# PaulMayer123/IMS-Toucan-Prosody-Variance

Hardware: AMD Instinct MI355X
Metric: mel-frames/sec + vocoder RTF @24kHz, batch=32, 1/2/4/8 MI355X (higher is better)
Workload: dtype bf16

## Files before the change

ims-toucan-prosody-variance_amd/csrc/common.h:

```cpp
#pragma once
#include <hip/hip_runtime.h>
#include <stdint.h>
#include <stdio.h>

#include "../../include/toucan_tts.h"

namespace tts {

void set_error(const char* fmt, ...);

#define TTS_CHECK_ARG(cond, ...)   \
  do {                             \
    if (!(cond)) {                 \
      tts::set_error(__VA_ARGS__); \
      return TTS_E_ARG;            \
    }                              \
  } while (0)

inline int launch_status(const char* what) {
  hipError_t e = hipGetLastError();
  if (e != hipSuccess) {
    set_error("%s: %s", what, hipGetErrorString(e));
    return TTS_E_LAUNCH;
  }
  return TTS_OK;
}

inline hipError_t raise_lds_limit(const void* kernel, unsigned long long& mask) {
  int dev = 0;
  (void)hipGetDevice(&dev);
  const unsigned long long bit = 1ull << (dev & 63);
  if (mask & bit) return hipSuccess;
  int room = 160 * 1024;
  hipFuncAttributes attr;
  if (hipFuncGetAttributes(&attr, kernel) == hipSuccess) room -= (int)attr.sharedSizeBytes;
  else (void)hipGetLastError();
  const hipError_t e = hipFuncSetAttribute(kernel, hipFuncAttributeMaxDynamicSharedMemorySize, room);
  if (e == hipSuccess) mask |= bit;
  else (void)hipGetLastError();
  return e;
}

struct WavenetCond {
  const float* g;
  int ld_g;
  const void* wc;
  int wc_n;
  int col0;
  const float* bc;
};
int wavenet_layer_cond(const TtsWavenetDesc& d, const WavenetCond& c, hipStream_t st);

typedef float f32x16 __attribute__((ext_vector_type(16)));
typedef float f32x4 __attribute__((ext_vector_type(4)));
typedef short bf16x8 __attribute__((ext_vector_type(8)));

__device__ __forceinline__ unsigned short f32_to_bf16(float f) {
  const __bf16 b = (__bf16)f;
  return __builtin_bit_cast(unsigned short, b);
}
__device__ __forceinline__ float bf16_to_f32(unsigned short u) { return __builtin_bit_cast(float, (unsigned int)u << 16); }

typedef _Float16 f16x2 __attribute__((ext_vector_type(2)));
typedef __bf16 bf16x2 __attribute__((ext_vector_type(2)));
typedef _Float16 f16x8 __attribute__((ext_vector_type(8)));
typedef float f32x2 __attribute__((ext_vector_type(2)));
__device__ __forceinline__ unsigned short f32_to_f16(float f) { return __builtin_bit_cast(unsigned short, (_Float16)f); }
__device__ __forceinline__ float f16_to_f32(unsigned short u) { return (float)__builtin_bit_cast(_Float16, u); }
template <bool F16>
__device__ __forceinline__ unsigned short to16(float f) {
  if constexpr (F16) return f32_to_f16(f);
  else return f32_to_bf16(f);
}
template <bool F16>
__device__ __forceinline__ float from16(unsigned short u) {
  if constexpr (F16) return f16_to_f32(u);
  else return bf16_to_f32(u);
}
template <bool F16>
__device__ __forceinline__ unsigned int pack16(float lo, float hi) {
  const f32x2 v = {lo, hi};
  if constexpr (F16) return __builtin_bit_cast(unsigned int, __builtin_convertvector(v, f16x2));
  else return __builtin_bit_cast(unsigned int, __builtin_convertvector(v, bf16x2));
}
__device__ __forceinline__ float load16(unsigned short u, bool f16) { return f16 ? f16_to_f32(u) : bf16_to_f32(u); }
__device__ __forceinline__ unsigned short store16(float v, bool f16) { return f16 ? f32_to_f16(v) : f32_to_bf16(v); }

template <bool F16>
__device__ __forceinline__ f32x16 mfma16(bf16x8 a, bf16x8 b, f32x16 c) {
  if constexpr (F16) return __builtin_amdgcn_mfma_f32_32x32x16_f16(__builtin_bit_cast(f16x8, a), __builtin_bit_cast(f16x8, b), c, 0, 0, 0);
  else return __builtin_amdgcn_mfma_f32_32x32x16_bf16(a, b, c, 0, 0, 0);
}

#define TTS_GLOAD128(dst_, ptr_) asm volatile("global_load_dwordx4 %0, %1, off" : "=v"(dst_) : "v"(ptr_) : "memory")
#define TTS_GLOAD32(dst_, ptr_) asm volatile("global_load_dword %0, %1, off" : "=v"(dst_) : "v"(ptr_) : "memory")
#define TTS_WAIT_VM(n_) asm volatile("s_waitcnt vmcnt(%0)" ::"n"(n_) : "memory")
#define TTS_PIN(r_) asm volatile("" : "+v"(r_))

__device__ __forceinline__ float sigmoidf_(float v) { return 1.0f / (1.0f + __expf(-v)); }

__device__ __forceinline__ float wave_sum(float v) {
#pragma unroll
  for (int o = 32; o > 0; o >>= 1) v += __shfl_xor(v, o, 64);
  return v;
}

__device__ __forceinline__ float wave_max(float v) {
#pragma unroll
  for (int o = 32; o > 0; o >>= 1) v = fmaxf(v, __shfl_xor(v, o, 64));
  return v;
}

}
```

ims-toucan-prosody-variance_amd/csrc/pipeline.hip:

```cpp
#include <algorithm>
#include <cmath>
#include <cstdlib>
#include <cstring>
#include <string>
#include <unordered_map>
#include <utility>
#include <vector>

#include "common.h"
#include "../../include/toucan_prosody.h"
#include "../../include/toucan_prosody_curves.h"
#include "../../include/toucan_score.h"

namespace tts {

const char* conv1d_wide_reject(const TtsConvDesc& d);

namespace {

constexpr int ATT = 192, HEADS = 4, DK = 48;

struct Dev {
  void* p = nullptr;
  int64_t shape[4] = {0, 0, 0, 0};
// ... 1095 lines not shown

int pipeline_teacher_forced(Handle* h, const float* gold_pitch, const float* gold_energy, const int* gold_dur, float* pred_log_dur,
                            float* pred_pitch, float* pred_energy, int* frames_out, hipStream_t st) {
  TTS_CHECK_ARG(h && h->enc, "tts_teacher_forced: run tts_encoder first");
  TTS_CHECK_RESOLVED(h, "tts_teacher_forced");
  TTS_CHECK_ARG(gold_pitch && gold_energy && gold_dur && pred_log_dur && pred_pitch && pred_energy, "tts_teacher_forced: null pointer");
  h->split_mode = 2;
  h->tab_which = 0;
  const Acoustic& m = h->acoustic;
  const int R = h->lp.total;
  if (h->cfg.multispeaker) TTS_TRY(cln_prepare(h, st));
  TTS_TRY(predictor(h, m.pitch, pred_pitch, st));
  TTS_TRY(predictor(h, m.energy, pred_energy, st));
  TTS_TRY(predictor(h, m.duration, pred_log_dur, st));
  TTS_TRY(hip_ok(hipMemcpyAsync(h->pitch, gold_pitch, (size_t)R * 4, hipMemcpyDeviceToDevice, st), "gold pitch"));
  TTS_TRY(hip_ok(hipMemcpyAsync(h->energy, gold_energy, (size_t)R * 4, hipMemcpyDeviceToDevice, st), "gold energy"));
  TTS_TRY(hip_ok(hipMemcpyAsync(h->dur, gold_dur, (size_t)R * 4, hipMemcpyDeviceToDevice, st), "gold durations"));
  return regulate(h, gold_dur, true, frames_out, st);
}

int pipeline_decoder(Handle* h, hipStream_t st) {
  TTS_CHECK_ARG(h && h->dec, "tts_decoder: run tts_control_and_regulate first");
  TTS_CHECK_RESOLVED(h, "tts_decoder");
  h->split_mode = 1;
  h->tab_which = 0;
  TTS_TRY(conformer(h, 1, h->dec, h->lf, h->frame, st));
  TTS_ALLOC(mel0, h->frame, float, (size_t)h->lf.total * 80);
  h->mel0 = mel0;
  h->mel = nullptr;
  return conv(h, h->acoustic.feat_out, T2(h->dec, ATT), T2(mel0, 80), h->lf, st);
}

int pipeline_postnet(Handle* h, hipStream_t st) {
  TTS_CHECK_ARG(h && h->mel0, "tts_postnet: run tts_decoder first");
  TTS_CHECK_RESOLVED(h, "tts_postnet");
  h->split_mode = 1;
  h->tab_which = 0;
  const Layout& l = h->lf;
  const int RF = l.total;
  Arena& a = h->frame;
  TTS_ALLOC(x, a, float, (size_t)RF * 256);
  TTS_ALLOC(y, a, float, (size_t)RF * 256);
  TTS_ALLOC(y80, a, float, (size_t)RF * 80);
  const long long wsn = std::max<long long>(1, tts_groupnorm_workspace_floats(l.n(), l.max_len, 32));
  TTS_ALLOC(gws, a, float, wsn);
  const int *sb, *se;
  TTS_TRY(bounds_of(h, l, st, &sb, &se));
  const float* src = h->mel0;
  int ld = 80;
  for (int i = 0; i < 5; ++i) {
    const auto& p = h->acoustic.postnet[i];
    if (i < 4) {
      TTS_TRY(conv(h, p.conv, T2(const_cast<float*>(src), ld), T2(x, 256), l, st));
      TTS_TRY(tts_groupnorm(x, 256, y, 256, p.g, p.b, 256, 32, 1e-5f, 1, nullptr, 0, sb, se, l.n(), l.max_len, gws, st));
      src = y;
      ld = 256;
    } else {
      TTS_TRY(conv(h, p.conv, T2(const_cast<float*>(src), ld), T2(y80, 80), l, st));
      TTS_TRY(tts_groupnorm(y80, 80, h->cat, 80 + ATT, p.g, p.b, 80, 20, 1e-5f, 0, h->mel0, 80, sb, se, l.n(), l.max_len, gws, st));
    }
  }
  h->mel = h->cat;
  h->have_flow = false;
  return TTS_OK;
}

int pipeline_postflow(Handle* h, const float* z_noise, hipStream_t st) {
  TTS_CHECK_ARG(h && h->mel == h->cat && h->cat, "tts_postflow: run tts_postnet first");
  TTS_CHECK_ARG(z_noise, "tts_postflow: z_noise is required");
  TTS_CHECK_RESOLVED(h, "tts_postflow");
  h->split_mode = 1;
  h->tab_which = 0;
  const Layout ls = h->lf.halved();
  const int RF = h->lf.total, RS = RF / 2;
  Arena& a = h->frame;
  const int b16 = bits16(h);
  const Acoustic& m = h->acoustic;
  TTS_ALLOC(g, a, float, (size_t)RF * ATT);
  TTS_TRY(conv(h, m.g_proj, T2(h->cat, 80 + ATT), T2(g, ATT), h->lf, st));
  TTS_ALLOC(x, a, float, (size_t)RS * 160);
  TTS_TRY(hip_ok(hipMemcpyAsync(x, z_noise, (size_t)RS * 160 * 4, hipMemcpyDeviceToDevice, st), "flow noise"));
  TTS_ALLOC(hs, a, float, (size_t)RS * 2 * ATT);
  const bool fused = !postflow_cond_buffer(h);
  float* hs2 = nullptr;
  TileTab t64;
  if (fused) {
    hs2 = arena_alloc<float>(a, (size_t)RS * 2 * ATT);
    if (!hs2) {
      set_error("tts_postflow: workspace exhausted");
      return TTS_E_ARG;
    }
    TTS_TRY(tiles_of(h, ls, 64, st, &t64));
  }
  char* acts = nullptr;
  float* cond = nullptr;
  if (!fused) {
    acts = arena_alloc<char>(a, (size_t)RS * ATT * (b16 / 8));
    cond = arena_alloc<float>(a, (size_t)RS * 8 * ATT);
    if (!acts || !cond) {
      set_error("tts_postflow: workspace exhausted");
      return TTS_E_ARG;
    }
  }
  float* skip = hs + ATT;
  double live_rows = 0;
  for (int n : ls.lengths) live_rows += n;
  for (int b = 17; b >= 0; --b) {
    const auto& f = m.flow[b];
    const ConvW& cnd = f.cond;
    TTS_TRY(conv(h, f.start, T2(x, 160), T2(hs, 2 * ATT), ls, st));
    if (!fused) TTS_TRY(conv(h, cnd, T2(g, 2 * ATT), T2(cond, 8 * ATT), ls, st));
    float* cur = hs;
    for (int i = 0; i < 4; ++i) {
      const ConvW &inl = m.flowgrp[b / 4].inl[i], &rs = m.flowgrp[b / 4].res_skip[i];
      if (fused) {
        float* nxt = cur == hs ? hs2 : hs;
        TtsWavenetDesc w;
        memset(&w, 0, sizeof(w));
        w.hs_in = cur; w.ld_in = 2 * ATT; w.hs_out = nxt; w.ld_out = 2 * ATT;
        w.w1 = inl.w16; w.b1 = inl.bias; w.w2 = rs.w16; w.b2 = rs.bias;
        w.cout2 = rs.cout; w.compute = inl.compute16;
        w.tiles = t64.dev; w.n_tiles = t64.n; w.tile_rows = 64;
        TTS_CHECK_ARG(cnd.w16 && cnd.mode == TTS_MODE_LINEAR && cnd.compute16 == inl.compute16 && cnd.cin == 2 * ATT && cnd.cin_pad == 2 * ATT && cnd.cout == 8 * ATT &&
                          cnd.taps == 1 && cnd.wn >= 8 * ATT,
                      "tts_postflow: flow.%d.cond is not a 16-bit 1-tap 384 -> 1536 conv", b);
        const WavenetCond wc = {g, 2 * ATT, cnd.w16, cnd.wn, i * 2 * ATT, cnd.bias};
        TTS_TRY(prof_launch(h, "wavenet_layer", 2.0 * live_rows * (ATT * 5 * 2 * ATT + 2 * ATT * 2 * ATT + (double)ATT * rs.cout),
                            live_rows * 4.0 * (2 * ATT + rs.cout + 2 * ATT) + 2.0 * (5 * ATT * 2 * ATT + 2 * ATT * 2 * ATT + ATT * rs.cout),
                            live_rows * rs.cout, st, [&] { return wavenet_layer_cond(w, wc, st); }));
        cur = nxt;
        continue;
      }
      ConvOpt oi;
      oi.preadd = cond + (size_t)i * 2 * ATT;
      oi.ld_preadd = 8 * ATT;
      TTS_TRY(conv(h, inl, T2(hs, 2 * ATT), T2(acts, ATT, b16), ls, st, oi));
      ConvOpt orr;
      orr.accumulate = true;
      TTS_TRY(conv(h, rs, T2(acts, ATT, b16), i < 3 ? T2(hs, 2 * ATT) : T2(skip, 2 * ATT), ls, st, orr));
    }
    ConvOpt oe;
    oe.aux = x + 80;
    oe.ld_aux = 160;
    oe.fp32_only = true;
    TTS_TRY(conv(h, f.end, T2(cur + ATT, 2 * ATT), T2(x + 80, 160), ls, st, oe));
    TTS_TRY(tts_glow_invconv_actnorm(x, 160, RS, 160, f.winv, f.an_bias, f.an_logs, st));
  }
  h->mel = x;
  h->have_flow = true;
  return TTS_OK;
}

struct ArenaRewind {
  Arena& a;
  size_t off;
  explicit ArenaRewind(Arena& a_) : a(a_), off(a_.off) {}
  ~ArenaRewind() { a.off = off; }
};

int pipeline_postflow_nll(Handle* h, const float* gold, int ld_gold, float* loss, float* row_parts, float* z_out, hipStream_t st) {
  TTS_CHECK_ARG(h, "tts_postflow_nll: null handle");
  TTS_CHECK_ARG(!is16(h), "tts_postflow_nll: fp32 handles only (this one was created with precision %d)", h->cfg.precision);
  TTS_CHECK_ARG(find(h, "flow.logdet") && find(h, "flow.0.wfwd") && find(h, "flow.0.end_ml.w"),
                "tts_postflow_nll: the forward weights flow.<b>.wfwd, flow.<b>.end_ml and flow.logdet were not loaded (tts_load_weights; "
                "NativePipeline(..., scoring=True) uploads them)");
  TTS_CHECK_ARG(h->mel == h->cat && h->cat, "tts_postflow_nll: run tts_postnet first");
  TTS_CHECK_ARG(gold && ld_gold >= 80 && loss, "tts_postflow_nll: null gold_mel / loss_out, or row stride %d < 80", ld_gold);
  TTS_CHECK_RESOLVED(h, "tts_postflow_nll");
  const Acoustic& m = h->acoustic;
  TTS_CHECK_ARG(m.scoring, "tts_postflow_nll: the forward weights were not resolved: run tts_encoder again");
  h->split_mode = 1;
  h->tab_which = 0;
  const Layout ls = h->lf.halved();
  const int RF = h->lf.total, RS = RF / 2, B = h->lf.n();
  long long live_rows = 0;
  for (int n : ls.lengths) live_rows += n;
  const size_t ml_bytes = ((size_t)RS * 160 * 4 + 255) & ~(size_t)255, ld_bytes = ((size_t)RS * 8 + 255) & ~(size_t)255;
  TTS_TRY(arena_reserve(h->nll, ml_bytes + ld_bytes, st));
  TTS_ALLOC(ml, h->nll, float, (size_t)RS * 160);
  TTS_ALLOC(row_logdet, h->nll, double, RS);
  TTS_TRY(hip_ok(hipMemsetAsync(h->nll.base, 0, ml_bytes + ld_bytes, st), "tts_postflow_nll: clear scratch"));
  void* tab;
  TTS_TRY(table_of(h, layout_key(h->lf, -2), st, [&] {
    std::vector<int> host(3 * (size_t)B);
    for (int u = 0; u < B; ++u) {
      host[u] = ls.begins[u];
      host[B + u] = ls.lengths[u];
      host[2 * B + u] = h->lf.lengths[u];
    }
    return host;
  }, &tab, nullptr));
  const int* utt = static_cast<const int*>(tab);
  Arena& a = h->frame;
  ArenaRewind rewind(a);
  TTS_ALLOC(x, a, float, (size_t)RS * 160);
  TTS_TRY(hip_ok(hipMemcpy2DAsync(x, 80 * 4, gold, (size_t)ld_gold * 4, 80 * 4, RF, hipMemcpyDeviceToDevice, st), "tts_postflow_nll: gold mel"));
  if (live_rows > 0) {
    TTS_ALLOC(g, a, float, (size_t)RF * ATT);
    TTS_TRY(conv(h, m.g_proj, T2(h->cat, 80 + ATT), T2(g, ATT), h->lf, st));
    TTS_ALLOC(hs, a, float, (size_t)RS * 2 * ATT);
    TTS_ALLOC(acts, a, float, (size_t)RS * ATT);
    TTS_ALLOC(cond, a, float, (size_t)RS * 8 * ATT);
    float* skip = hs + ATT;
    TTS_TRY(tts_glow_forward_rows(x, 160, RS, nullptr, 0, nullptr, m.flow_fwd[0].wfwd, m.flow[0].an_bias, m.flow[0].an_logs, st));
    for (int b = 0; b < 18; ++b) {
      const auto& f = m.flow[b];
      TTS_TRY(conv(h, f.start, T2(x, 160), T2(hs, 2 * ATT), ls, st));
      TTS_TRY(conv(h, f.cond, T2(g, 2 * ATT), T2(cond, 8 * ATT), ls, st));
      for (int i = 0; i < 4; ++i) {
        const ConvW &inl = m.flowgrp[b / 4].inl[i], &rs = m.flowgrp[b / 4].res_skip[i];
        ConvOpt oi;
        oi.preadd = cond + (size_t)i * 2 * ATT;
        oi.ld_preadd = 8 * ATT;
        TTS_TRY(conv(h, inl, T2(hs, 2 * ATT), T2(acts, ATT), ls, st, oi));
        ConvOpt orr;
        orr.accumulate = true;
        TTS_TRY(conv(h, rs, T2(acts, ATT), i < 3 ? T2(hs, 2 * ATT) : T2(skip, 2 * ATT), ls, st, orr));
      }
      ConvOpt oe;
      oe.fp32_only = true;
      TTS_TRY(conv(h, m.flow_fwd[b].end_ml, T2(skip, 2 * ATT), T2(ml, 160), ls, st, oe));
      const bool last = b == 17;
      TTS_TRY(tts_glow_forward_rows(x, 160, RS, ml, 160, row_logdet, last ? nullptr : m.flow_fwd[b + 1].wfwd, last ? nullptr : m.flow[b + 1].an_bias,
                                    last ? nullptr : m.flow[b + 1].an_logs, st));
    }
  }
  TTS_TRY(tts_glow_nll_reduce(x, 160, row_logdet, utt, utt + B, utt + 2 * B, B, m.flow_logdet, loss, row_parts, st));
  if (z_out) TTS_TRY(hip_ok(hipMemcpyAsync(z_out, x, (size_t)RS * 160 * 4, hipMemcpyDeviceToDevice, st), "tts_postflow_nll: z_out"));
// ... 369 lines not shown
```

ims-toucan-prosody-variance_amd/csrc/wavenet.hip:

```cpp
#include "common.h"

namespace tts {

namespace {
constexpr int WN_H = 192;
constexpr int WN_BM = 64;
constexpr int WN_TAPS = 5;
constexpr int WN_XP = WN_H + 8;
constexpr int WN_G = 2 * WN_H;
constexpr int WN_GP = WN_G + 8;
constexpr int WN_STEPS1 = WN_TAPS * (WN_H / 16);
constexpr int WN_STEPSC = WN_G / 16;
constexpr int WN_STEPS2 = WN_H / 16;
constexpr int WN_DEPTH = 4;
constexpr int WN_L = 4;
constexpr size_t WN_XS_BYTES = ((size_t)(WN_BM + WN_TAPS - 1) * WN_XP * 2 + 255) / 256 * 256;
constexpr size_t WN_GS_BYTES = (size_t)WN_BM * WN_GP * 2;
static_assert(WN_STEPS1 % WN_DEPTH == 0 && WN_STEPSC % WN_DEPTH == 0 && WN_STEPS2 % WN_DEPTH == 0 && (WN_H / 16) % WN_DEPTH == 0,
              "a block of WN_DEPTH k-steps stays inside one tap and one product");
}

template <bool F16, bool FUSED>
__global__ __launch_bounds__(256) void wavenet_layer_kernel(const TtsWavenetDesc d, const WavenetCond cd) {
  extern __shared__ __attribute__((aligned(16))) unsigned char lds_raw[];
// ... 166 lines not shown
          }
        } else {
          const float4 ea = *reinterpret_cast<const float4*>(cr + c), eg = *reinterpret_cast<const float4*>(cr + WN_H + c);
          pa[0] = ea.x; pa[1] = ea.y; pa[2] = ea.z; pa[3] = ea.w;
          pg[0] = eg.x; pg[1] = eg.y; pg[2] = eg.z; pg[3] = eg.w;
        }
        const float bav[4] = {ba.x, ba.y, ba.z, ba.w}, bgv[4] = {bg.x, bg.y, bg.z, bg.w};
        float v[4];
#pragma unroll
        for (int q = 0; q < 4; ++q) {
          const float av = aa[4 * rq + q] + bav[q] + pa[q], gvv = ag[4 * rq + q] + bgv[q] + pg[q];
          const float th = 2.0f * __builtin_amdgcn_rcpf(1.0f + __expf(-2.0f * av)) - 1.0f;
          v[q] = th * __builtin_amdgcn_rcpf(1.0f + __expf(-gvv));
        }
        *reinterpret_cast<uint2*>(xs + t * WN_XP + c) = make_uint2(pack16<F16>(v[0], v[1]), pack16<F16>(v[2], v[3]));
      }
    };
    constexpr int CZ = FUSED ? 1 : 0;
    gate(acc[0], acc[2], accc[0 * CZ], accc[2 * CZ], P0, fP);
    gate(acc[1], acc[3], accc[1 * CZ], accc[3 * CZ], P0, fQ);
    gate(acc[4], acc[5], accc[4 * CZ], accc[5 * CZ], P1, fP);
#pragma unroll
    for (int j = 0; j < 6; ++j)
#pragma unroll
      for (int r = 0; r < 16; ++r) acc[j][r] = 0.0f;
  }
  publish();
  xload(xP, xQ, xs, WN_XP);
#pragma unroll 1
  for (int base = 0; base < WN_STEPS2; base += WN_DEPTH) {
    if (base == WN_STEPS2 - WN_DEPTH) {
      q0 -= qs; q1 -= qs; q2 -= qs; q3 -= qs;
      qs = 0;
    }
#pragma unroll
    for (int u = 0; u < WN_DEPTH; ++u) {
      const bf16x8 cP = xP, cQ = xQ;
      const int s1 = base + u + 1 < WN_STEPS2 ? base + u + 1 : WN_STEPS2 - 1;
      xload(xP, xQ, xs + s1 * 16, WN_XP);
      arrive(u);
      u32x4 wf[3];
#pragma unroll
      for (int i = 0; i < 3; ++i) wf[i] = wr[u][i];
      acc[0] = mfma16<F16>(__builtin_bit_cast(bf16x8, wf[0]), cP, acc[0]);
      acc[1] = mfma16<F16>(__builtin_bit_cast(bf16x8, wf[0]), cQ, acc[1]);
      acc[2] = mfma16<F16>(__builtin_bit_cast(bf16x8, wf[1]), cP, acc[2]);
      if (n2 == 384) {
        acc[3] = mfma16<F16>(__builtin_bit_cast(bf16x8, wf[1]), cQ, acc[3]);
        acc[4] = mfma16<F16>(__builtin_bit_cast(bf16x8, wf[2]), cP, acc[4]);
        acc[5] = mfma16<F16>(__builtin_bit_cast(bf16x8, wf[2]), cQ, acc[5]);
      }
      request(u);
    }
  }
  TTS_WAIT_VM(0);
#pragma unroll
  for (int u = 0; u < WN_DEPTH; ++u) {
    TTS_PIN(wr[u][0]);
    TTS_PIN(wr[u][1]);
    TTS_PIN(wr[u][2]);
    TTS_PIN(wr[u][3]);
  }
  {
    const int col0 = n2 == 384 ? 0 : WN_H;
    auto store_block = [&](const f32x16& a, int cb, int f) __attribute__((always_inline)) {
      const int row = tile.row0 + f * 32 + lrow;
      if (row >= tile.seq_end) return;
      const float* ir = d.hs_in + (size_t)row * d.ld_in + col0;
      float* orow = d.hs_out + (size_t)row * d.ld_out + col0;
#pragma unroll
      for (int rq = 0; rq < 4; ++rq) {
        const int c = cb * 32 + 8 * rq + 4 * lk;
        const float4 b = *reinterpret_cast<const float4*>(d.b2 + c), x = *reinterpret_cast<const float4*>(ir + c);
        *reinterpret_cast<float4*>(orow + c) = make_float4((a[4 * rq] + b.x) + x.x, (a[4 * rq + 1] + b.y) + x.y, (a[4 * rq + 2] + b.z) + x.z, (a[4 * rq + 3] + b.w) + x.w);
      }
    };
    store_block(acc[0], cb0, fP);
    store_block(acc[1], cb0, fQ);
    store_block(acc[2], cb1, fP);
    if (n2 == 384) {
      store_block(acc[3], cb1, fQ);
      store_block(acc[4], cb2, fP);
      store_block(acc[5], cb2, fQ);
    }
  }
}

namespace {
int wavenet_launch(const TtsWavenetDesc& d, const WavenetCond* c, hipStream_t st) {
  TTS_CHECK_ARG(d.hs_in && d.hs_out && d.w1 && d.b1 && d.w2 && d.b2 && d.tiles, "wavenet_layer: null pointer");
  TTS_CHECK_ARG(d.hs_in != d.hs_out, "wavenet_layer: the hidden state cannot be updated in place (the 5-tap conv reads neighbouring tiles)");
  TTS_CHECK_ARG(d.cout2 == 384 || d.cout2 == 192, "wavenet_layer: res/skip width %d (384, or 192 for the last layer)", d.cout2);
  TTS_CHECK_ARG(d.compute == TTS_COMPUTE_BF16 || d.compute == TTS_COMPUTE_F16, "wavenet_layer: 16-bit MFMA configurations only (compute %d)", d.compute);
  TTS_CHECK_ARG(d.tile_rows == WN_BM, "wavenet_layer: tile table must use %d rows, got %d", WN_BM, d.tile_rows);
  TTS_CHECK_ARG((d.ld_in & 3) == 0 && (d.ld_out & 3) == 0 && ((uintptr_t)d.hs_in & 15) == 0 && ((uintptr_t)d.hs_out & 15) == 0 && ((uintptr_t)d.w1 & 15) == 0 &&
                    ((uintptr_t)d.w2 & 15) == 0 && ((uintptr_t)d.b1 & 15) == 0 && ((uintptr_t)d.b2 & 15) == 0,
                "wavenet_layer: rows and weights must be 16-byte aligned");
  if (c) {
    TTS_CHECK_ARG(c->g && c->wc && c->bc, "wavenet_layer: null conditioning pointer");
    TTS_CHECK_ARG(c->ld_g >= WN_G && (c->ld_g & 3) == 0 && c->col0 >= 0 && (c->col0 & 31) == 0 && c->col0 + 2 * WN_H <= c->wc_n,
                  "wavenet_layer: conditioning columns %d .. of %d, row stride %d", c->col0, c->wc_n, c->ld_g);
    TTS_CHECK_ARG(((uintptr_t)c->g & 15) == 0 && ((uintptr_t)c->wc & 15) == 0 && ((uintptr_t)c->bc & 15) == 0, "wavenet_layer: conditioning operands must be 16-byte aligned");
  } else {
    TTS_CHECK_ARG(d.cond, "wavenet_layer: null pointer");
    TTS_CHECK_ARG((d.ld_cond & 3) == 0 && ((uintptr_t)d.cond & 15) == 0, "wavenet_layer: rows and weights must be 16-byte aligned");
  }
  if (d.n_tiles == 0) return TTS_OK;
  const bool f16 = d.compute == TTS_COMPUTE_F16;
  const WavenetCond none = {nullptr, 0, nullptr, 0, 0, nullptr};
  if (c) {
    const size_t lds = WN_XS_BYTES + WN_GS_BYTES;
    static unsigned long long raised[2] = {0, 0};
    const void* k = f16 ? reinterpret_cast<const void*>(wavenet_layer_kernel<true, true>) : reinterpret_cast<const void*>(wavenet_layer_kernel<false, true>);
    if (raise_lds_limit(k, raised[f16 ? 1 : 0]) != hipSuccess) {
      set_error("wavenet_layer: raising the dynamic LDS limit failed");
      return TTS_E_LAUNCH;
    }
    if (f16) hipLaunchKernelGGL((wavenet_layer_kernel<true, true>), dim3(d.n_tiles), dim3(256), lds, st, d, *c);
    else hipLaunchKernelGGL((wavenet_layer_kernel<false, true>), dim3(d.n_tiles), dim3(256), lds, st, d, *c);
  } else {
    if (f16) hipLaunchKernelGGL((wavenet_layer_kernel<true, false>), dim3(d.n_tiles), dim3(256), WN_XS_BYTES, st, d, none);
    else hipLaunchKernelGGL((wavenet_layer_kernel<false, false>), dim3(d.n_tiles), dim3(256), WN_XS_BYTES, st, d, none);
  }
  return launch_status("wavenet_layer");
}
}

int wavenet_layer(const TtsWavenetDesc& d, hipStream_t st) { return wavenet_launch(d, nullptr, st); }

int wavenet_layer_cond(const TtsWavenetDesc& d, const WavenetCond& c, hipStream_t st) { return wavenet_launch(d, &c, st); }

}

extern "C" int tts_wavenet_layer(const TtsWavenetDesc* d, tts_stream_t stream) {
  if (!d) {
    tts::set_error("tts_wavenet_layer: null descriptor");
    return TTS_E_ARG;
  }
  return tts::wavenet_layer(*d, reinterpret_cast<hipStream_t>(stream));
}
```

Before: 595,300.

## Fuse flow start conv and four WaveNet layers into one halo-tiled block kernel

Replaces the per-layer WaveNet launches (start conv plus four conditioned layers with ping-pong hidden buffers) with a single kernel per flow step. Each block computes 64 rows and stores the middle 48, relying on an 8-row halo on each side to cover the receptive field of the four 5-tap convs. The hidden state stays in registers and LDS across layers, and only the skip output is written to global memory. This removes the intermediate hidden-state round trips and launch overhead. In exchange it recomputes the halo rows (16 of every 64, about a third extra work per output row) and raises register and LDS pressure.

```diff
diff --git a/ims-toucan-prosody-variance_amd/csrc/common.h b/ims-toucan-prosody-variance_amd/csrc/common.h
--- a/ims-toucan-prosody-variance_amd/csrc/common.h
+++ b/ims-toucan-prosody-variance_amd/csrc/common.h
@@ -50,6 +50,20 @@
   const float* bc;
 };
 int wavenet_layer_cond(const TtsWavenetDesc& d, const WavenetCond& c, hipStream_t st);
+
+struct WavenetBlock {
+  const float* x; int ld_x;
+  float* skip; int ld_skip;
+  const void* w0; int w0_n; const float* b0;
+  const void* w1[4]; const float* b1[4];
+  const void* w2[4]; const float* b2[4];
+  const float* g; int ld_g;
+  const void* wc; int wc_n; const float* bc;
+  const TtsTile* tiles; int n_tiles; int tile_rows;
+  int compute;
+};
+int wavenet_block(const WavenetBlock& d, hipStream_t st);
+int wavenet_block_tile_rows();
 
 typedef float f32x16 __attribute__((ext_vector_type(16)));
 typedef float f32x4 __attribute__((ext_vector_type(4)));
diff --git a/ims-toucan-prosody-variance_amd/csrc/pipeline.hip b/ims-toucan-prosody-variance_amd/csrc/pipeline.hip
--- a/ims-toucan-prosody-variance_amd/csrc/pipeline.hip
+++ b/ims-toucan-prosody-variance_amd/csrc/pipeline.hip
@@ -1201,16 +1201,8 @@
   TTS_TRY(hip_ok(hipMemcpyAsync(x, z_noise, (size_t)RS * 160 * 4, hipMemcpyDeviceToDevice, st), "flow noise"));
   TTS_ALLOC(hs, a, float, (size_t)RS * 2 * ATT);
   const bool fused = !postflow_cond_buffer(h);
-  float* hs2 = nullptr;
-  TileTab t64;
-  if (fused) {
-    hs2 = arena_alloc<float>(a, (size_t)RS * 2 * ATT);
-    if (!hs2) {
-      set_error("tts_postflow: workspace exhausted");
-      return TTS_E_ARG;
-    }
-    TTS_TRY(tiles_of(h, ls, 64, st, &t64));
-  }
+  TileTab tblk;
+  if (fused) TTS_TRY(tiles_of(h, ls, wavenet_block_tile_rows(), st, &tblk));
   char* acts = nullptr;
   float* cond = nullptr;
   if (!fused) {
@@ -1227,29 +1219,33 @@
   for (int b = 17; b >= 0; --b) {
     const auto& f = m.flow[b];
     const ConvW& cnd = f.cond;
-    TTS_TRY(conv(h, f.start, T2(x, 160), T2(hs, 2 * ATT), ls, st));
-    if (!fused) TTS_TRY(conv(h, cnd, T2(g, 2 * ATT), T2(cond, 8 * ATT), ls, st));
-    float* cur = hs;
-    for (int i = 0; i < 4; ++i) {
+    if (!fused) {
+      TTS_TRY(conv(h, f.start, T2(x, 160), T2(hs, 2 * ATT), ls, st));
+      TTS_TRY(conv(h, cnd, T2(g, 2 * ATT), T2(cond, 8 * ATT), ls, st));
+    }
+    if (fused) {
+      TTS_CHECK_ARG(f.start.w16 && f.start.mode == TTS_MODE_LINEAR && f.start.compute16 == cnd.compute16 && f.start.cin == 80 && f.start.taps == 1 && f.start.wn >= ATT,
+                    "tts_postflow: flow.%d.start is not a 16-bit 1-tap 80 -> 192 conv", b);
+      TTS_CHECK_ARG(cnd.w16 && cnd.mode == TTS_MODE_LINEAR && cnd.cin == 2 * ATT && cnd.cin_pad == 2 * ATT && cnd.cout == 8 * ATT && cnd.taps == 1 && cnd.wn >= 8 * ATT,
+                    "tts_postflow: flow.%d.cond is not a 16-bit 1-tap 384 -> 1536 conv", b);
+      WavenetBlock w;
+      memset(&w, 0, sizeof(w));
+      w.x = x; w.ld_x = 160; w.skip = skip; w.ld_skip = 2 * ATT;
+      w.w0 = f.start.w16; w.w0_n = f.start.wn; w.b0 = f.start.bias;
+      w.g = g; w.ld_g = 2 * ATT; w.wc = cnd.w16; w.wc_n = cnd.wn; w.bc = cnd.bias;
+      w.tiles = tblk.dev; w.n_tiles = tblk.n; w.tile_rows = wavenet_block_tile_rows();
+      w.compute = cnd.compute16;
+      for (int i = 0; i < 4; ++i) {
+        const ConvW &inl = m.flowgrp[b / 4].inl[i], &rs = m.flowgrp[b / 4].res_skip[i];
+        TTS_CHECK_ARG(inl.w16 && rs.w16 && inl.compute16 == cnd.compute16 && rs.cout == (i < 3 ? 2 * ATT : ATT), "tts_postflow: flow.%d layer %d is not a 16-bit WaveNet layer", b, i);
+        w.w1[i] = inl.w16; w.b1[i] = inl.bias; w.w2[i] = rs.w16; w.b2[i] = rs.bias;
+      }
+      TTS_TRY(prof_launch(h, "wavenet_block", 2.0 * live_rows * (80.0 * ATT + 4.0 * (ATT * 5 * 2 * ATT + 2 * ATT * 2 * ATT) + 3.0 * ATT * 2 * ATT + (double)ATT * ATT),
+                          live_rows * 4.0 * (80 + ATT + 2 * ATT) + 2.0 * (80.0 * ATT + 4.0 * (5 * ATT * 2 * ATT + 2 * ATT * 2 * ATT) + 3.0 * ATT * 2 * ATT + (double)ATT * ATT),
+                          live_rows * ATT, st, [&] { return wavenet_block(w, st); }));
+    }
+    for (int i = 0; i < 4 && !fused; ++i) {
       const ConvW &inl = m.flowgrp[b / 4].inl[i], &rs = m.flowgrp[b / 4].res_skip[i];
-      if (fused) {
-        float* nxt = cur == hs ? hs2 : hs;
-        TtsWavenetDesc w;
-        memset(&w, 0, sizeof(w));
-        w.hs_in = cur; w.ld_in = 2 * ATT; w.hs_out = nxt; w.ld_out = 2 * ATT;
-        w.w1 = inl.w16; w.b1 = inl.bias; w.w2 = rs.w16; w.b2 = rs.bias;
-        w.cout2 = rs.cout; w.compute = inl.compute16;
-        w.tiles = t64.dev; w.n_tiles = t64.n; w.tile_rows = 64;
-        TTS_CHECK_ARG(cnd.w16 && cnd.mode == TTS_MODE_LINEAR && cnd.compute16 == inl.compute16 && cnd.cin == 2 * ATT && cnd.cin_pad == 2 * ATT && cnd.cout == 8 * ATT &&
-                          cnd.taps == 1 && cnd.wn >= 8 * ATT,
-                      "tts_postflow: flow.%d.cond is not a 16-bit 1-tap 384 -> 1536 conv", b);
-        const WavenetCond wc = {g, 2 * ATT, cnd.w16, cnd.wn, i * 2 * ATT, cnd.bias};
-        TTS_TRY(prof_launch(h, "wavenet_layer", 2.0 * live_rows * (ATT * 5 * 2 * ATT + 2 * ATT * 2 * ATT + (double)ATT * rs.cout),
-                            live_rows * 4.0 * (2 * ATT + rs.cout + 2 * ATT) + 2.0 * (5 * ATT * 2 * ATT + 2 * ATT * 2 * ATT + ATT * rs.cout),
-                            live_rows * rs.cout, st, [&] { return wavenet_layer_cond(w, wc, st); }));
-        cur = nxt;
-        continue;
-      }
       ConvOpt oi;
       oi.preadd = cond + (size_t)i * 2 * ATT;
       oi.ld_preadd = 8 * ATT;
@@ -1262,7 +1258,7 @@
     oe.aux = x + 80;
     oe.ld_aux = 160;
     oe.fp32_only = true;
-    TTS_TRY(conv(h, f.end, T2(cur + ATT, 2 * ATT), T2(x + 80, 160), ls, st, oe));
+    TTS_TRY(conv(h, f.end, T2(skip, 2 * ATT), T2(x + 80, 160), ls, st, oe));
     TTS_TRY(tts_glow_invconv_actnorm(x, 160, RS, 160, f.winv, f.an_bias, f.an_logs, st));
   }
   h->mel = x;
diff --git a/ims-toucan-prosody-variance_amd/csrc/wavenet.hip b/ims-toucan-prosody-variance_amd/csrc/wavenet.hip
--- a/ims-toucan-prosody-variance_amd/csrc/wavenet.hip
+++ b/ims-toucan-prosody-variance_amd/csrc/wavenet.hip
@@ -272,6 +272,286 @@
       store_block(acc[3], cb1, fQ);
       store_block(acc[4], cb2, fP);
       store_block(acc[5], cb2, fQ);
+    }
+  }
+}
+
+namespace {
+constexpr int WB_OUT = 48;
+constexpr int WB_HALO = 8;
+constexpr int WB_CIN = 80;
+constexpr size_t WB_AS_BYTES = (size_t)WN_BM * WN_XP * 2;
+constexpr size_t WB_LDS_BYTES = WN_XS_BYTES + WB_AS_BYTES + WN_GS_BYTES;
+static_assert(WB_OUT + 2 * WB_HALO == WN_BM, "stored rows plus the halo are the computed tile");
+}
+
+template <bool F16>
+__global__ __launch_bounds__(256) void wavenet_block_kernel(const WavenetBlock d) {
+  extern __shared__ __attribute__((aligned(16))) unsigned char lds_raw[];
+  unsigned short* xs = reinterpret_cast<unsigned short*>(lds_raw);
+  unsigned short* as = reinterpret_cast<unsigned short*>(lds_raw + WN_XS_BYTES);
+  unsigned short* gs = reinterpret_cast<unsigned short*>(lds_raw + WN_XS_BYTES + WB_AS_BYTES);
+  const TtsTile tile = d.tiles[blockIdx.x];
+  const int c0 = tile.row0 - WB_HALO;
+  const int tid = threadIdx.x, lane = tid & 63, lrow = lane & 31, lk = lane >> 5;
+  const int wave = __builtin_amdgcn_readfirstlane(tid >> 6);
+  const int P0 = (wave * 5 + 1) / 3, P1 = wave < 2 ? 1 : 4, fP = wave & 1, fQ = fP ^ 1;
+  auto clamp_row = [&](int gr) __attribute__((always_inline)) { return gr < tile.seq_begin ? tile.seq_begin : (gr >= tile.seq_end ? tile.seq_end - 1 : gr); };
+  auto pick = [&](auto (&arr)[4], int i) __attribute__((always_inline)) { return i == 0 ? arr[0] : (i == 1 ? arr[1] : (i == 2 ? arr[2] : arr[3])); };
+
+  typedef unsigned int u32x4 __attribute__((ext_vector_type(4)));
+  u32x4 wr[WN_DEPTH][WN_L];
+  const char *q0, *q1, *q2, *q3;
+  size_t qs;
+  auto request = [&](int slot) __attribute__((always_inline)) {
+    TTS_GLOAD128(wr[slot][0], q0);
+    TTS_GLOAD128(wr[slot][1], q1);
+    TTS_GLOAD128(wr[slot][2], q2);
+    TTS_GLOAD128(wr[slot][3], q3);
+    q0 += qs; q1 += qs; q2 += qs; q3 += qs;
+  };
+  auto arrive = [&](int slot) __attribute__((always_inline)) {
+    TTS_WAIT_VM((WN_DEPTH - 1) * WN_L);
+    TTS_PIN(wr[slot][0]);
+    TTS_PIN(wr[slot][1]);
+    TTS_PIN(wr[slot][2]);
+    TTS_PIN(wr[slot][3]);
+  };
+  auto stream_pairs = [&](const void* w, int n, int col0) __attribute__((always_inline)) {
+    const char* b = reinterpret_cast<const char*>(w) + ((size_t)lk * n + col0 + lrow) * 16;
+    q0 = b + P0 * 512; q1 = q0 + WN_H * 16; q2 = b + P1 * 512; q3 = q2 + WN_H * 16;
+    qs = (size_t)n * 32;
+  };
+  auto stream_res_skip = [&](const void* w, int n, int cb) __attribute__((always_inline)) {
+    const char* b = reinterpret_cast<const char*>(w) + ((size_t)lk * n + lrow) * 16 + cb * 512;
+    q0 = b; q1 = b + 512; q2 = b + 1024; q3 = q2;
+    qs = (size_t)n * 32;
+  };
+  auto publish = [&]() __attribute__((always_inline)) {
+    asm volatile("s_waitcnt lgkmcnt(0)" ::: "memory");
+    __builtin_amdgcn_s_barrier();
+  };
+
+  stream_pairs(d.w1[0], 2 * WN_H, 0);
+#pragma unroll
+  for (int u = 0; u < WN_DEPTH; ++u) request(u);
+
+  {
+    constexpr int GQ4 = WN_G / 4, GPER = WN_BM * GQ4 / 256, PER = 8;
+    static_assert(GPER % PER == 0, "g staging trips");
+#pragma unroll 1
+    for (int p0 = 0; p0 < GPER; p0 += PER) {
+      float4 v[PER];
+#pragma unroll
+      for (int p = 0; p < PER; ++p) {
+        const int e = tid + (p0 + p) * 256, r = e / GQ4, c4 = (e % GQ4) * 4;
+        v[p] = *reinterpret_cast<const float4*>(d.g + (size_t)clamp_row(c0 + r) * d.ld_g + c4);
+      }
+#pragma unroll
+      for (int p = 0; p < PER; ++p) {
+        const int e = tid + (p0 + p) * 256, r = e / GQ4, c4 = (e % GQ4) * 4;
+        *reinterpret_cast<uint2*>(gs + r * WN_GP + c4) = make_uint2(pack16<F16>(v[p].x, v[p].y), pack16<F16>(v[p].z, v[p].w));
+      }
+    }
+  }
+  f32x16 st[6];
+#pragma unroll
+  for (int j = 0; j < 6; ++j)
+#pragma unroll
+    for (int r = 0; r < 16; ++r) st[j][r] = 0.0f;
+  if (wave < 2) {
+    const float* xrP = d.x + (size_t)clamp_row(c0 + fP * 32 + lrow) * d.ld_x + lk * 8;
+    const float* xrQ = d.x + (size_t)clamp_row(c0 + fQ * 32 + lrow) * d.ld_x + lk * 8;
+    const char* wb = reinterpret_cast<const char*>(d.w0) + ((size_t)lk * d.w0_n + 96 * wave + lrow) * 16;
+#pragma unroll
+    for (int s = 0; s < WB_CIN / 16; ++s) {
+      const float4 p0 = *reinterpret_cast<const float4*>(xrP + 16 * s), p1 = *reinterpret_cast<const float4*>(xrP + 16 * s + 4);
+      const float4 r0 = *reinterpret_cast<const float4*>(xrQ + 16 * s), r1 = *reinterpret_cast<const float4*>(xrQ + 16 * s + 4);
+      const u32x4 uP = {pack16<F16>(p0.x, p0.y), pack16<F16>(p0.z, p0.w), pack16<F16>(p1.x, p1.y), pack16<F16>(p1.z, p1.w)};
+      const u32x4 uQ = {pack16<F16>(r0.x, r0.y), pack16<F16>(r0.z, r0.w), pack16<F16>(r1.x, r1.y), pack16<F16>(r1.z, r1.w)};
+#pragma unroll
+      for (int i = 0; i < 3; ++i) {
+        const u32x4 wf = *reinterpret_cast<const u32x4*>(wb + (size_t)s * d.w0_n * 32 + i * 512);
+        st[2 * i] = mfma16<F16>(__builtin_bit_cast(bf16x8, wf), __builtin_bit_cast(bf16x8, uP), st[2 * i]);
+        st[2 * i + 1] = mfma16<F16>(__builtin_bit_cast(bf16x8, wf), __builtin_bit_cast(bf16x8, uQ), st[2 * i + 1]);
+      }
+    }
+#pragma unroll
+    for (int j = 0; j < 6; ++j) {
+      const int cb = 3 * wave + (j >> 1), t = ((j & 1) ? fQ : fP) * 32 + lrow, gr = c0 + t;
+      const bool inside = gr >= tile.seq_begin && gr < tile.seq_end;
+#pragma unroll
+      for (int rq = 0; rq < 4; ++rq) {
+        const int c = cb * 32 + 8 * rq + 4 * lk;
+        const float4 b = *reinterpret_cast<const float4*>(d.b0 + c);
+        const float v0 = (st[j][4 * rq] + b.x) + 0.0f, v1 = (st[j][4 * rq + 1] + b.y) + 0.0f;
+        const float v2 = (st[j][4 * rq + 2] + b.z) + 0.0f, v3 = (st[j][4 * rq + 3] + b.w) + 0.0f;
+        st[j][4 * rq] = v0; st[j][4 * rq + 1] = v1; st[j][4 * rq + 2] = v2; st[j][4 * rq + 3] = v3;
+        *reinterpret_cast<uint2*>(xs + (t + 2) * WN_XP + c) = inside ? make_uint2(pack16<F16>(v0, v1), pack16<F16>(v2, v3)) : make_uint2(0u, 0u);
+      }
+    }
+  } else {
+    constexpr int Q4 = WN_XP / 4;
+    for (int e = tid - 128; e < 4 * Q4; e += 128) {
+      const int r = e / Q4, row = r < 2 ? r : WN_BM + r;
+      *reinterpret_cast<uint2*>(xs + row * WN_XP + (e % Q4) * 4) = make_uint2(0u, 0u);
+    }
+  }
+
+  f32x16 acc[6], accc[6];
+  auto xload = [&](bf16x8& xP, bf16x8& xQ, const unsigned short* xrow, int pitch) __attribute__((always_inline)) {
+    xP = *reinterpret_cast<const bf16x8*>(xrow + (fP * 32 + lrow) * pitch + lk * 8);
+    xQ = *reinterpret_cast<const bf16x8*>(xrow + (fQ * 32 + lrow) * pitch + lk * 8);
+  };
+  auto pair_step = [&](int slot, f32x16 (&a)[6], bf16x8& xP, bf16x8& xQ, const unsigned short* xnext, int pitch) __attribute__((always_inline)) {
+    const bf16x8 cP = xP, cQ = xQ;
+    xload(xP, xQ, xnext, pitch);
+    arrive(slot);
+    u32x4 wf[WN_L];
+#pragma unroll
+    for (int i = 0; i < WN_L; ++i) wf[i] = wr[slot][i];
+    a[0] = mfma16<F16>(__builtin_bit_cast(bf16x8, wf[0]), cP, a[0]);
+    a[1] = mfma16<F16>(__builtin_bit_cast(bf16x8, wf[0]), cQ, a[1]);
+    a[2] = mfma16<F16>(__builtin_bit_cast(bf16x8, wf[1]), cP, a[2]);
+    a[3] = mfma16<F16>(__builtin_bit_cast(bf16x8, wf[1]), cQ, a[3]);
+    a[4] = mfma16<F16>(__builtin_bit_cast(bf16x8, wf[2]), cP, a[4]);
+    a[5] = mfma16<F16>(__builtin_bit_cast(bf16x8, wf[3]), cP, a[5]);
+    request(slot);
+  };
+  bf16x8 xP, xQ;
+  auto window_at = [&](int s) __attribute__((always_inline)) {
+    s = s < WN_STEPS1 ? s : WN_STEPS1 - 1;
+    return xs + (s / (WN_H / 16)) * WN_XP + (s % (WN_H / 16)) * 16;
+  };
+
+#pragma unroll 1
+  for (int i = 0; i < 4; ++i) {
+    const float *b1 = pick(d.b1, i), *b2 = pick(d.b2, i);
+    const void* w2 = pick(d.w2, i);
+    const int n2 = i < 3 ? 2 * WN_H : WN_H, cbase = i < 3 ? 3 * wave : 3 * (wave & 1), ccol = i * 2 * WN_H;
+    publish();
+#pragma unroll
+    for (int j = 0; j < 6; ++j)
+#pragma unroll
+      for (int r = 0; r < 16; ++r) acc[j][r] = 0.0f;
+    xload(xP, xQ, window_at(0), WN_XP);
+#pragma unroll 1
+    for (int base = 0; base < WN_STEPS1; base += WN_DEPTH) {
+      if (base == WN_STEPS1 - WN_DEPTH) stream_pairs(d.wc, d.wc_n, ccol);
+#pragma unroll
+      for (int u = 0; u < WN_DEPTH; ++u) pair_step(u, acc, xP, xQ, window_at(base + u + 1), WN_XP);
+    }
+#pragma unroll
+    for (int j = 0; j < 6; ++j)
+#pragma unroll
+      for (int r = 0; r < 16; ++r) accc[j][r] = 0.0f;
+    xload(xP, xQ, gs, WN_GP);
+#pragma unroll 1
+    for (int base = 0; base < WN_STEPSC; base += WN_DEPTH) {
+      if (base == WN_STEPSC - WN_DEPTH) stream_res_skip(w2, n2, cbase);
+#pragma unroll
+      for (int u = 0; u < WN_DEPTH; ++u) {
+        const int s1 = base + u + 1 < WN_STEPSC ? base + u + 1 : WN_STEPSC - 1;
+        pair_step(u, accc, xP, xQ, gs + s1 * 16, WN_GP);
+      }
+    }
+    {
+      auto gate = [&](const f32x16& aa, const f32x16& ag, const f32x16& ca, const f32x16& cg, int pb, int f) __attribute__((always_inline)) {
+        const int t = f * 32 + lrow;
+#pragma unroll
+        for (int rq = 0; rq < 4; ++rq) {
+          const int c = pb * 32 + 8 * rq + 4 * lk;
+          const float4 ba = *reinterpret_cast<const float4*>(b1 + c), bg = *reinterpret_cast<const float4*>(b1 + WN_H + c);
+          float pa[4], pg[4];
+          const float4 ea = *reinterpret_cast<const float4*>(d.bc + ccol + c), eg = *reinterpret_cast<const float4*>(d.bc + ccol + WN_H + c);
+          const float eav[4] = {ea.x, ea.y, ea.z, ea.w}, egv[4] = {eg.x, eg.y, eg.z, eg.w};
+#pragma unroll
+          for (int q = 0; q < 4; ++q) {
+            pa[q] = (ca[4 * rq + q] + eav[q]) + 0.0f;
+            pg[q] = (cg[4 * rq + q] + egv[q]) + 0.0f;
+          }
+          const float bav[4] = {ba.x, ba.y, ba.z, ba.w}, bgv[4] = {bg.x, bg.y, bg.z, bg.w};
+          float v[4];
+#pragma unroll
+          for (int q = 0; q < 4; ++q) {
+            const float av = aa[4 * rq + q] + bav[q] + pa[q], gvv = ag[4 * rq + q] + bgv[q] + pg[q];
+            const float th = 2.0f * __builtin_amdgcn_rcpf(1.0f + __expf(-2.0f * av)) - 1.0f;
+            v[q] = th * __builtin_amdgcn_rcpf(1.0f + __expf(-gvv));
+          }
+          *reinterpret_cast<uint2*>(as + t * WN_XP + c) = make_uint2(pack16<F16>(v[0], v[1]), pack16<F16>(v[2], v[3]));
+        }
+      };
+      gate(acc[0], acc[2], accc[0], accc[2], P0, fP);
+      gate(acc[1], acc[3], accc[1], accc[3], P0, fQ);
+      gate(acc[4], acc[5], accc[4], accc[5], P1, fP);
+#pragma unroll
+      for (int j = 0; j < 6; ++j)
+#pragma unroll
+        for (int r = 0; r < 16; ++r) acc[j][r] = 0.0f;
+    }
+    publish();
+    xload(xP, xQ, as, WN_XP);
+#pragma unroll 1
+    for (int base = 0; base < WN_STEPS2; base += WN_DEPTH) {
+      if (base == WN_STEPS2 - WN_DEPTH) {
+        if (i < 3) {
+          stream_pairs(pick(d.w1, i + 1), 2 * WN_H, 0);
+        } else {
+          q0 -= qs; q1 -= qs; q2 -= qs; q3 -= qs;
+          qs = 0;
+        }
+      }
+#pragma unroll
+      for (int u = 0; u < WN_DEPTH; ++u) {
+        const bf16x8 cP = xP, cQ = xQ;
+        const int s1 = base + u + 1 < WN_STEPS2 ? base + u + 1 : WN_STEPS2 - 1;
+        xload(xP, xQ, as + s1 * 16, WN_XP);
+        arrive(u);
+        u32x4 wf[3];
+#pragma unroll
+        for (int k = 0; k < 3; ++k) wf[k] = wr[u][k];
+        acc[0] = mfma16<F16>(__builtin_bit_cast(bf16x8, wf[0]), cP, acc[0]);
+        acc[1] = mfma16<F16>(__builtin_bit_cast(bf16x8, wf[0]), cQ, acc[1]);
+        acc[2] = mfma16<F16>(__builtin_bit_cast(bf16x8, wf[1]), cP, acc[2]);
+        acc[3] = mfma16<F16>(__builtin_bit_cast(bf16x8, wf[1]), cQ, acc[3]);
+        acc[4] = mfma16<F16>(__builtin_bit_cast(bf16x8, wf[2]), cP, acc[4]);
+        acc[5] = mfma16<F16>(__builtin_bit_cast(bf16x8, wf[2]), cQ, acc[5]);
+        request(u);
+      }
+    }
+#pragma unroll
+    for (int j = 0; j < 6; ++j) {
+      const int cb = cbase + (j >> 1), t = ((j & 1) ? fQ : fP) * 32 + lrow, gr = c0 + t;
+      const bool inside = gr >= tile.seq_begin && gr < tile.seq_end;
+#pragma unroll
+      for (int rq = 0; rq < 4; ++rq) {
+        const int c = cb * 32 + 8 * rq + 4 * lk;
+        const float4 b = *reinterpret_cast<const float4*>(b2 + c);
+        const float v0 = (acc[j][4 * rq] + b.x) + st[j][4 * rq], v1 = (acc[j][4 * rq + 1] + b.y) + st[j][4 * rq + 1];
+        const float v2 = (acc[j][4 * rq + 2] + b.z) + st[j][4 * rq + 2], v3 = (acc[j][4 * rq + 3] + b.w) + st[j][4 * rq + 3];
+        st[j][4 * rq] = v0; st[j][4 * rq + 1] = v1; st[j][4 * rq + 2] = v2; st[j][4 * rq + 3] = v3;
+        if (i < 3 && wave < 2)
+          *reinterpret_cast<uint2*>(xs + (t + 2) * WN_XP + c) = inside ? make_uint2(pack16<F16>(v0, v1), pack16<F16>(v2, v3)) : make_uint2(0u, 0u);
+      }
+    }
+  }
+  TTS_WAIT_VM(0);
+#pragma unroll
+  for (int u = 0; u < WN_DEPTH; ++u) {
+    TTS_PIN(wr[u][0]);
+    TTS_PIN(wr[u][1]);
+    TTS_PIN(wr[u][2]);
+    TTS_PIN(wr[u][3]);
+  }
+  if (wave >= 2) {
+#pragma unroll
+    for (int j = 0; j < 6; ++j) {
+      const int cb = 3 * (wave - 2) + (j >> 1), t = ((j & 1) ? fQ : fP) * 32 + lrow, row = c0 + t;
+      if (t < WB_HALO || t >= WB_HALO + WB_OUT || row >= tile.seq_end) continue;
+      float* orow = d.skip + (size_t)row * d.ld_skip + cb * 32 + 4 * lk;
+#pragma unroll
+      for (int rq = 0; rq < 4; ++rq)
+        *reinterpret_cast<float4*>(orow + 8 * rq) = make_float4(st[j][4 * rq], st[j][4 * rq + 1], st[j][4 * rq + 2], st[j][4 * rq + 3]);
     }
   }
 }
@@ -316,6 +596,36 @@
 }
 }
 
+int wavenet_block_tile_rows() { return WB_OUT; }
+
+int wavenet_block(const WavenetBlock& d, hipStream_t st) {
+  TTS_CHECK_ARG(d.x && d.w0 && d.b0 && d.skip && d.g && d.wc && d.bc && d.tiles, "wavenet_block: null pointer");
+  for (int i = 0; i < 4; ++i) {
+    TTS_CHECK_ARG(d.w1[i] && d.b1[i] && d.w2[i] && d.b2[i], "wavenet_block: null weights of layer %d", i);
+    TTS_CHECK_ARG(((uintptr_t)d.w1[i] & 15) == 0 && ((uintptr_t)d.w2[i] & 15) == 0 && ((uintptr_t)d.b1[i] & 15) == 0 && ((uintptr_t)d.b2[i] & 15) == 0,
+                  "wavenet_block: weights must be 16-byte aligned");
+  }
+  TTS_CHECK_ARG(d.compute == TTS_COMPUTE_BF16 || d.compute == TTS_COMPUTE_F16, "wavenet_block: 16-bit MFMA configurations only (compute %d)", d.compute);
+  TTS_CHECK_ARG(d.tile_rows == WB_OUT, "wavenet_block: tile table must use %d rows, got %d", WB_OUT, d.tile_rows);
+  TTS_CHECK_ARG(d.ld_x >= WB_CIN && (d.ld_x & 3) == 0 && d.ld_skip >= WN_H && (d.ld_skip & 3) == 0 && d.ld_g >= WN_G && (d.ld_g & 3) == 0 &&
+                    ((uintptr_t)d.x & 15) == 0 && ((uintptr_t)d.skip & 15) == 0 && ((uintptr_t)d.g & 15) == 0 && ((uintptr_t)d.wc & 15) == 0 && ((uintptr_t)d.bc & 15) == 0 &&
+                    ((uintptr_t)d.w0 & 15) == 0 && ((uintptr_t)d.b0 & 15) == 0,
+                "wavenet_block: rows, start and conditioning operands must be 16-byte aligned");
+  TTS_CHECK_ARG(d.w0_n >= WN_H, "wavenet_block: the start conv has %d packed columns, the hidden state %d", d.w0_n, WN_H);
+  TTS_CHECK_ARG(d.wc_n >= 8 * WN_H, "wavenet_block: %d conditioning columns, four layers need %d", d.wc_n, 8 * WN_H);
+  if (d.n_tiles == 0) return TTS_OK;
+  const bool f16 = d.compute == TTS_COMPUTE_F16;
+  static unsigned long long raised[2] = {0, 0};
+  const void* k = f16 ? reinterpret_cast<const void*>(wavenet_block_kernel<true>) : reinterpret_cast<const void*>(wavenet_block_kernel<false>);
+  if (raise_lds_limit(k, raised[f16 ? 1 : 0]) != hipSuccess) {
+    set_error("wavenet_block: raising the dynamic LDS limit failed");
+    return TTS_E_LAUNCH;
+  }
+  if (f16) hipLaunchKernelGGL((wavenet_block_kernel<true>), dim3(d.n_tiles), dim3(256), WB_LDS_BYTES, st, d);
+  else hipLaunchKernelGGL((wavenet_block_kernel<false>), dim3(d.n_tiles), dim3(256), WB_LDS_BYTES, st, d);
+  return launch_status("wavenet_block");
+}
+
 int wavenet_layer(const TtsWavenetDesc& d, hipStream_t st) { return wavenet_launch(d, nullptr, st); }
 
 int wavenet_layer_cond(const TtsWavenetDesc& d, const WavenetCond& c, hipStream_t st) { return wavenet_launch(d, &c, st); }
```

After: 615,500 (median of 6 runs). +3.4%, better.
